# AbeelLab/phasm

Hardware: AMD Instinct MI355X
Metric: overlaps_per_sec (higher is better)
Workload: dtype u64

## Files before the change

phasm_amd/csrc/c_api.hip:

```cpp
#include "../../include/phasm_overlap.h"

#include <hip/hip_runtime.h>

#include <dlfcn.h>
#include <execinfo.h>
#include <fcntl.h>
#include <signal.h>
#include <sys/mman.h>
#include <sys/stat.h>
#include <unistd.h>

#include <algorithm>
#include <array>
#include <atomic>
#include <chrono>
#include <cmath>
#include <condition_variable>
#include <cstdio>
#include <cstdlib>
#include <cstring>
#include <deque>
#include <functional>
#include <memory>
#include <mutex>
// ... 610 lines not shown


unsigned cpu_share() {
    static const unsigned share = [] {
        unsigned n = std::thread::hardware_concurrency();
        n = n ? n : 4u;
        long long q = -1, per = 100000;
        if (FILE* f = std::fopen("/sys/fs/cgroup/cpu.max", "r")) {
            char buf[64] = {0};
            if (std::fscanf(f, "%63s %lld", buf, &per) >= 1 && std::strcmp(buf, "max") != 0) q = atoll(buf);
            std::fclose(f);
        } else if (FILE* g = std::fopen("/sys/fs/cgroup/cpu/cpu.cfs_quota_us", "r")) {
            if (std::fscanf(g, "%lld", &q) != 1) q = -1;
            std::fclose(g);
            if (FILE* g2 = std::fopen("/sys/fs/cgroup/cpu/cpu.cfs_period_us", "r")) {
                if (std::fscanf(g2, "%lld", &per) != 1) per = 100000;
                std::fclose(g2);
            }
        }
        if (q > 0 && per > 0) n = std::min<unsigned>(n, (unsigned)std::max<long long>(1, q / per));
        return n;
    }();
    return share;
}

namespace home {

constexpr uint32_t CHUNK = 4096;

struct Job {
    const void* rec = nullptr;
    uint32_t sh_b = 0, sh_p = 0;
    uint64_t n_rec = 0;
    po_row* out = nullptr;
    uint64_t n_rows = 0;
    const volatile uint32_t* flag = nullptr;
    uint32_t want = 0;
    uint32_t paired = 0, bits = 2;
};

struct Pool {
    std::vector<std::thread> thr;
    std::mutex mu;
    std::condition_variable cv_queue;
    std::condition_variable cv_job;
    std::mutex call_mu;
    std::deque<Job> queue;
    std::atomic<uint64_t> submitted{0}, finished{0};
    std::atomic<int> error{0};
    const uint32_t* len = nullptr;
    uint32_t n_reads = 0;
    std::atomic<uint64_t> sum_l{0}, sum_b{0}, sum_e{0};
    Job cur;
    uint64_t job_seq = 0;
    uint32_t n_chunks = 0;
    std::vector<uint64_t> chunk_off;
    std::atomic<uint32_t> next_count{0}, done_count{0}, next_write{0}, done_write{0};
    std::atomic<int> phase{0};
    std::atomic<int> inside{0};
    std::chrono::steady_clock::time_point t0;
    std::vector<std::array<double, 3>> trace;
    bool tracing = false;
};

Pool* g_pool = nullptr;
std::once_flag g_pool_once;

inline void cpu_pause() {
#if defined(__x86_64__) || defined(__i386__)
    __builtin_ia32_pause();
#endif
}

std::atomic<uint32_t> g_spin_limit{4096};
template <class Pred>
inline void spin_until(Pred pred) {
    const uint32_t limit = g_spin_limit.load(std::memory_order_relaxed);
    for (uint32_t n = 0; !pred(); ++n) {
        if (limit == 0 || n < limit) cpu_pause();
        else std::this_thread::yield();
    }
}

inline po::Cand load_rec(const Job& j, uint64_t i) {
    if (!j.sh_b) return static_cast<const po::Cand*>(j.rec)[i];
    return po::unpack_record(static_cast<const uint64_t*>(j.rec)[i], j.sh_b, j.sh_p);
}

inline uint32_t rows_of_rec(const po::Cand& c, uint32_t paired) {
    if (!paired) return (c.type & 1u) + ((c.type >> 1) & 1u);
    return ((c.type & 1u) ? (c.a == (c.b ^ 1u) ? 1u : 2u) : 0u) + ((c.type & 2u) ? 2u : 0u);
}

inline void put_row(uint64_t*& o, uint32_t a, uint32_t b, uint32_t astart, uint32_t aend, uint32_t bend) {
    __builtin_nontemporal_store((uint64_t)a | ((uint64_t)b << 32), o);
    __builtin_nontemporal_store((uint64_t)astart | ((uint64_t)aend << 32), o + 1);
    __builtin_nontemporal_store((uint64_t)bend << 32, o + 2);
    o += 3;
}

bool expand_records(Pool& P, uint64_t lo, uint64_t hi, po_row* out) {
    uint64_t* o = reinterpret_cast<uint64_t*>(out);
    const Job& job = P.cur;
    const uint32_t* len = P.len;
    const uint32_t paired = job.paired, n_reads = P.n_reads, bits = job.bits;
    auto pb = [bits](uint32_t l) -> uint64_t { return bits == 8u ? l : (l >> 2) + ((l & 3u) != 0u); };
    uint64_t sl = 0, sb = 0, se = 0;
    for (uint64_t i = lo; i < hi; ++i) {
        const po::Cand c = load_rec(job, i);
        if (c.a >= n_reads || c.b >= n_reads) return false;
        const uint32_t la = len[c.a], lb = len[c.b];
        se += 2 * pb((c.type & 1u) ? la - c.p : lb);
        if (c.type & 1u) {
            const uint32_t l = la - c.p;
            const bool twin = paired && c.a != (c.b ^ 1u);
            put_row(o, c.a, c.b, c.p, la, l);
            if (twin) put_row(o, c.b ^ 1u, c.a ^ 1u, lb - l, lb, l);
            const uint64_t k = twin ? 2 : 1;
            sl += k * l;
            sb += k * 2 * pb(l);
        }
        if (c.type & 2u) {
            put_row(o, c.a, c.b, c.p, c.p + lb, lb);
            if (paired) put_row(o, c.a ^ 1u, c.b ^ 1u, la - c.p - lb, la - c.p, lb);
            const uint64_t k = paired ? 2 : 1;
            sl += k * lb;
            sb += k * 2 * pb(lb);
        }
    }
    P.sum_l.fetch_add(sl, std::memory_order_relaxed);
    P.sum_b.fetch_add(sb, std::memory_order_relaxed);
    P.sum_e.fetch_add(se, std::memory_order_relaxed);
    return true;
}

void run_phases(Pool& P, bool lead) {
    const uint32_t nc = P.n_chunks;
    for (;;) {
        const uint32_t c = P.next_count.fetch_add(1, std::memory_order_relaxed);
        if (c >= nc) break;
        const uint64_t lo = (uint64_t)c * CHUNK, hi = std::min<uint64_t>(P.cur.n_rec, lo + CHUNK);
        uint64_t n = 0;
        const uint32_t paired = P.cur.paired;
        for (uint64_t i = lo; i < hi; ++i) n += rows_of_rec(load_rec(P.cur, i), paired);
        P.chunk_off[c + 1] = n;
        P.done_count.fetch_add(1, std::memory_order_release);
    }
    if (lead) {
        spin_until([&] { return P.done_count.load(std::memory_order_acquire) >= nc; });
        P.chunk_off[0] = 0;
        for (uint32_t c = 0; c < nc; ++c) P.chunk_off[c + 1] += P.chunk_off[c];
        if (P.chunk_off[nc] != P.cur.n_rows) P.error.store(1);
        P.phase.store(P.error.load() ? 0 : 2, std::memory_order_release);
    } else {
        spin_until([&] { return P.phase.load(std::memory_order_acquire) != 1; });
    }
    if (P.phase.load(std::memory_order_acquire) != 2) return;
    for (;;) {
        const uint32_t c = P.next_write.fetch_add(1, std::memory_order_relaxed);
        if (c >= nc) break;
        const uint64_t lo = (uint64_t)c * CHUNK, hi = std::min<uint64_t>(P.cur.n_rec, lo + CHUNK);
        if (!expand_records(P, lo, hi, P.cur.out + P.chunk_off[c])) P.error.store(2);
#if defined(__x86_64__)
        __builtin_ia32_sfence();
#endif
        P.done_write.fetch_add(1, std::memory_order_release);
    }
}

void helper(Pool* Pp) {
    Pool& P = *Pp;
    uint64_t seen = 0;
    for (;;) {
        {
            std::unique_lock<std::mutex> lock(P.mu);
            P.cv_job.wait(lock, [&] { return P.job_seq != seen; });
            seen = P.job_seq;
        }
        P.inside.fetch_add(1, std::memory_order_acq_rel);
        if (P.phase.load(std::memory_order_acquire) != 0) run_phases(P, false);
        P.inside.fetch_sub(1, std::memory_order_release);
    }
}

void leader(Pool* Pp) {
    Pool& P = *Pp;
    for (;;) {
        Job j;
        {
            std::unique_lock<std::mutex> lock(P.mu);
            P.cv_queue.wait(lock, [&] { return !P.queue.empty(); });
            j = P.queue.front();
            P.queue.pop_front();
        }
        if (j.flag)
            spin_until([&] { return *j.flag == j.want; });
        std::atomic_thread_fence(std::memory_order_acquire);
        const double t_ready = P.tracing ? std::chrono::duration<double, std::micro>(std::chrono::steady_clock::now() - P.t0).count() : 0.0;
        if (P.error.load() == 0 && j.n_rec) {
            spin_until([&] { return P.inside.load(std::memory_order_acquire) == 0; });
            P.cur = j;
            P.n_chunks = (uint32_t)((j.n_rec + CHUNK - 1) / CHUNK);
            if (P.chunk_off.size() < (size_t)P.n_chunks + 1) P.chunk_off.resize((size_t)P.n_chunks + 1);
            P.next_count.store(0);
            P.done_count.store(0);
            P.next_write.store(0);
            P.done_write.store(0);
            P.phase.store(1, std::memory_order_release);
            {
                std::lock_guard<std::mutex> lock(P.mu);
                ++P.job_seq;
            }
            P.cv_job.notify_all();
            run_phases(P, true);
            if (P.phase.load() == 2)
                spin_until([&] { return P.done_write.load(std::memory_order_acquire) >= P.n_chunks; });
            P.phase.store(0, std::memory_order_release);
            std::atomic_thread_fence(std::memory_order_seq_cst);
        }
        if (P.tracing)
            P.trace.push_back({t_ready, std::chrono::duration<double, std::micro>(std::chrono::steady_clock::now() - P.t0).count(), (double)j.n_rows});
        P.finished.fetch_add(1, std::memory_order_release);
    }
}

Pool* pool() {
    std::call_once(g_pool_once, [] {
        Pool* P = new Pool();
        unsigned n = cpu_share();
        n = std::max(1u, std::min(n * 3 / 4, 12u));
        if (const char* e = getenv("PHASM_HOME_THREADS")) n = (unsigned)std::max(1, std::min(64, atoi(e)));
        try {
            P->thr.emplace_back(leader, P);
            P->thr.back().detach();
            for (unsigned i = 1; i < n; ++i) {
                P->thr.emplace_back(helper, P);
                P->thr.back().detach();
            }
        } catch (const std::system_error&) {
        }
        if (P->thr.empty()) {
            delete P;
            P = nullptr;
        }
        g_pool = P;
    });
    return g_pool;
}

void begin(Pool* P, const uint32_t* len, uint32_t n_reads, bool tracing) {
    if (const char* e = getenv("PHASM_HOME_SPIN")) g_spin_limit.store((uint32_t)std::max(0, atoi(e)));
    else g_spin_limit.store(4096);
    P->len = len;
    P->n_reads = n_reads;
    P->error.store(0);
    P->submitted.store(0);
    P->finished.store(0);
    P->sum_l.store(0);
    P->sum_b.store(0);
    P->sum_e.store(0);
    P->tracing = tracing;
    P->trace.clear();
    P->t0 = std::chrono::steady_clock::now();
}

void submit(Pool* P, const Job& j) {
    {
        std::lock_guard<std::mutex> lock(P->mu);
        P->queue.push_back(j);
    }
    P->submitted.fetch_add(1, std::memory_order_release);
    P->cv_queue.notify_one();
}

void wait_all(Pool* P) {
    spin_until([&] { return P->finished.load(std::memory_order_acquire) >= P->submitted.load(std::memory_order_acquire); });
}

}

po_status init_device(po_handle* h) {
    if (h->dev_ready) {
        HIP_TRY(h, hipSetDevice(h->device));
        return PO_OK;
    }
    AllocTrace tr("init_device", 0);
    const auto ti0 = std::chrono::steady_clock::now();
    auto imark = [&](const char* what) {
        if (tr.on) std::fprintf(stderr, "[init] %s at %.1f ms\n", what, std::chrono::duration<double, std::milli>(std::chrono::steady_clock::now() - ti0).count());
    };
    int n = 0;
    hipError_t e = hipGetDeviceCount(&n);
    imark("runtime up (hipGetDeviceCount)");
    if (e != hipSuccess || n == 0)
        return fail(h, PO_ERR_HIP, "no HIP device available (libphasm_overlap has no CPU fallback)");
    if (h->device < 0 || h->device >= n) return fail(h, PO_ERR_INVALID, "device ordinal out of range");
    HIP_TRY(h, hipSetDevice(h->device));
    hipDeviceProp_t prop;
    HIP_TRY(h, hipGetDeviceProperties(&prop, h->device));
    h->n_cu = prop.multiProcessorCount > 0 ? prop.multiProcessorCount : 256;
// ... 934 lines not shown
            hipLaunchKernelGGL(k_cfill, dim3(cdiv(n_entries, 256)), dim3(256), 0, st, read_slot, entry_off,
                               (uint64_t)n_entries, slot_start, slot_cur, chain64, len);
            sort_chains<uint64_t>();
            hipLaunchKernelGGL(k_fin, dim3(cdiv(nslots, 256)), dim3(256), 0, st, table, nslots, slot_cnt,
                               slot_start, chain64, len);
        }
        HIP_TRY(h, hipGetLastError());
        if (phase_events) HIP_TRY(h, hipEventRecord(h->ev[EV_INDEX], st));
        if (slice_build) {
            HIP_TRY(h, hipStreamSynchronize(st));
            h->sl_tbits = tbits;
            h->sl_entries = h->pinned[0];
            if (phase_events) (void)hipEventElapsedTime(&S.ms_index, h->ev[EV_START], h->ev[EV_INDEX]);
            return PO_OK;
        }
        h->idx_valid = a.idx_only || !ext_idx;
        h->idx_gen = h->upload_gen;
        h->idx_m = m;
        h->idx_wide = wide;
        h->idx_tbits = tbits;
        h->idx_bits = (uint32_t)BITS;
        h->idx_ww = ww;
        *done = a.idx_only;
        return PO_OK;
    }

    po_status scan_count() {
        A.words = words;
        A.tiles = h->d_tiles.as<po::TileRec>();
        A.tile_begin = tile_begin;
        A.tile_end = tile_end;
        A.m = m;
        A.kmask = kmask;
        A.bloom = bloom;
        A.bloom_log2 = bloom_log2;
        A.table = table;
        A.tbits = tbits;
        A.chain = chain;
        A.len = len;
        A.paired = paired;
        A.selfrep = selfrep;
        A.n_selfrep = reinterpret_cast<uint32_t*>(scalars + 2);
        A.tile_count = h->d_tile_count.as<uint32_t>();
        A.tile_off = tile_off_p;
        A.truemask = h->d_truemask.as<uint32_t>();
#ifdef PO_STAMPS
        PO_TRY(ws(h->d_flag, (size_t)4096 * 64));
        HIP_TRY(h, hipMemsetAsync(h->d_flag.p, 0, (size_t)4096 * 64, st));
        A.dbg = h->d_flag.as<unsigned long long>();
#endif
        WA.words = words;
        WA.tiles = A.tiles;
        WA.tile_begin = tile_begin;
        WA.tile_end = tile_end;
        WA.m = m;
        WA.table = table;
        WA.tbits = tbits;
        WA.chain = h->d_chain.as<uint64_t>();
        WA.n_slices = 1;
        if (ext_idx) {
            WA.table = static_cast<const po::Slot*>(a.ext_index);
            WA.chain = nullptr;
            WA.n_slices = a.ext_slices;
            WA.chunk_slots = a.ext_chunk_slots;
            WA.chain_off_slots = a.ext_chain_off;
        }
        WA.len = len;
        WA.paired = paired;
        WA.tile_count = A.tile_count;
        WA.lane_slot = A.truemask;
        WA.tile_off = A.tile_off;
        if (wide) {
            if (pair_events) HIP_TRY(h, hipEventRecord(h->ev[EV_PROBE0], st));
            auto wscan = a.streamed ? (ww == 4 ? po::k_wide_scan<BITS, false, BITS == 2, 4> : po::k_wide_scan<BITS, false, BITS == 2, 1>)
                         : ww == 16 ? po::k_wide_scan<BITS, false, false, 16> : ww == 4 ? po::k_wide_scan<BITS, false, false, 4> : po::k_wide_scan<BITS, false, false, 1>;
            hipLaunchKernelGGL(wscan, dim3(cdiv(ntiles, 4)), dim3(256), 0, st, WA, po::CandGuard{nullptr, 0u});
            if (pair_events) HIP_TRY(h, hipEventRecord(h->ev[EV_PROBE1], st));
        } else {
            const size_t scan_lds = (size_t)scan_waves * po::SCAN_LDS_PER_WAVE + bloom_bytes;
            if (scan_lds > h->lds_max) return fail(h, PO_ERR_HIP, "device LDS too small for the scan kernel");
            constexpr bool CAN_STREAM = BITS == 2;
            auto probe_full = a.streamed ? po::k_scan_probe<BITS, true, CAN_STREAM> : po::k_scan_probe<BITS, true, false>;
            auto probe_part = a.streamed ? po::k_scan_probe<BITS, false, CAN_STREAM> : po::k_scan_probe<BITS, false, false>;
            HIP_TRY(h, hipFuncSetAttribute(reinterpret_cast<const void*>(probe_full), hipFuncAttributeMaxDynamicSharedMemorySize, (int)scan_lds));
            HIP_TRY(h, hipFuncSetAttribute(reinterpret_cast<const void*>(probe_part), hipFuncAttributeMaxDynamicSharedMemorySize, (int)scan_lds));
            const uint32_t n_scan_waves = scan_grid * scan_waves;
            PO_TRY(ws(h->d_left, (size_t)n_scan_waves * po::LEFT_CAP * sizeof(uint2)));
            PO_TRY(ws(h->d_left_cnt, (size_t)n_scan_waves * 4));
            PO_TRY(ws(h->d_tile_extra, ((size_t)h->n_tiles + 1) * 4));
            if (fold_clear && self_clean && h->st_selfclean) {
            } else if (fold_clear) {
                const uint32_t te0 = self_clean ? 0u : tile_begin, ten = self_clean ? h->n_tiles : ntiles;
                hipLaunchKernelGGL(po::k_call_reset, dim3(cdiv(std::max(std::max(n, 16u), std::max(n_scan_waves, ten)), 256)), dim3(256), 0, st,
                                   selfrep, n, self_clean ? h->d_scalars.as<unsigned long long>() : scalars, self_clean ? 16u : 8u,
                                   h->d_left_cnt.as<uint32_t>(), n_scan_waves, h->d_tile_extra.as<uint32_t>() + te0, ten);
            } else {
                HIP_TRY(h, hipMemsetAsync(h->d_left_cnt.p, 0, (size_t)n_scan_waves * 4, st));
                HIP_TRY(h, hipMemsetAsync(h->d_tile_extra.as<uint32_t>() + tile_begin, 0, (size_t)ntiles * 4, st));
            }
            A.left = h->d_left.as<uint2>();
            A.left_cnt = h->d_left_cnt.as<uint32_t>();
            A.tile_extra = h->d_tile_extra.as<uint32_t>();
            if (pair_events) HIP_TRY(h, hipEventRecord(h->ev[EV_PROBE0], st));
            hipLaunchKernelGGL(K == W ? probe_full : probe_part, dim3(scan_grid), dim3(scan_waves * 64), scan_lds, st, A);
            if (pair_events) HIP_TRY(h, hipEventRecord(h->ev[EV_PROBE1], st));
            auto fixup = a.streamed ? po::k_scan_fixup<BITS, CAN_STREAM> : po::k_scan_fixup<BITS, false>;
            hipLaunchKernelGGL(fixup, dim3(n_scan_waves), dim3(256), 0, st, A, n_scan_waves, self_clean ? 1u : 0u);
            if (sw.debug_left) {
                PO_TRY(ensure_host(h, h->scratch_host, (size_t)n_scan_waves * 4));
                HIP_TRY(h, hipMemcpyAsync(h->scratch_host.p, h->d_left_cnt.p, (size_t)n_scan_waves * 4, hipMemcpyDeviceToHost, st));
                HIP_TRY(h, hipStreamSynchronize(st));
                const uint32_t* lc = static_cast<const uint32_t*>(h->scratch_host.p);
                uint64_t sum = 0;
                uint32_t mx = 0;
                for (uint32_t k = 0; k < n_scan_waves; ++k) sum += lc[k], mx = std::max(mx, lc[k]);
                std::fprintf(stderr, "[left] %u scan waves deferred %llu positions (max %u per wave, cap %d)\n", n_scan_waves,
                             (unsigned long long)sum, mx, (int)po::LEFT_CAP);
            }
        }
        HIP_TRY(h, hipGetLastError());
#ifdef PO_STAMPS
        if (!wide) {
            std::vector<unsigned long long> dbg(4096 * 8);
            HIP_TRY(h, hipMemcpyAsync(dbg.data(), h->d_flag.p, dbg.size() * 8, hipMemcpyDeviceToHost, st));
            HIP_TRY(h, hipStreamSynchronize(st));
            double sum[6] = {0, 0, 0, 0, 0, 0};
            for (size_t w = 0; w < 4096; ++w) for (int k = 0; k < 6; ++k) sum[k] += (double)dbg[w * 8 + k];
            if (sum[5] > 0)
                std::fprintf(stderr, "[stamps] per pass (cycles): wait_rw %.0f  filter %.0f  wait_probe %.0f  consume %.0f  issue %.0f  (passes %.0f)\n",
                             sum[0] / sum[5], sum[1] / sum[5], sum[2] / sum[5], sum[3] / sum[5], sum[4] / sum[5], sum[5]);
        }
#endif
        return PO_OK;
    }

    po_status candidate_count() {
        if (a.streamed && h->st_harvest && h->st_pred_valid && !a.dp && !a.want_cands && !sw.sync_count && !sw.tail_classic) {
            uint64_t pred = h->st_pred_cand[a.shard];
            uint64_t cap = pred + pred / 50 + 256;
            if (sw.pred_scale) cap = pred = (uint64_t)((double)pred * atof(sw.pred_scale));
            const uint64_t worst = cap * 4u;
            bool order = pred >= 400000 && (r_end - r_begin) >= 4096;
            if (sw.verify_order) order = atoi(sw.verify_order) != 0;
            pred_order = order;
            auto fits = [](const DevBuf& b, uint64_t bytes) { return b.p && b.cap >= bytes; };
            async_count = pred > 0 && cap < (16u << 20) && cdiv(cap, po::TAIL_TILE) <= po::TAIL_MAX_TILES &&
                          fits(h->d_cand_a, cap * 4) && fits(h->d_cand_p, cap * 4) && fits(h->d_cand_b, cap * 4) && fits(h->d_type, cap) &&
                          fits(h->d_rowcnt, cap) && fits(h->d_row_off, (cap + 1) * 4) &&
                          fits(h->spare_rows, h->home_on ? cap * sizeof(po::Cand) : worst * sizeof(po_row)) &&
                          (!order || (fits(h->d_vlabel, (uint64_t)(r_end - r_begin) * 4) && fits(h->d_vperm, (uint64_t)(r_end - r_begin) * 4) &&
                                      fits(h->d_vrank, (uint64_t)(r_end - r_begin) * 4))) && h->dev_words < 0xFFFFFFF0ull;
            cap_c = (uint32_t)cap;
        }
        volatile uint64_t* count_slot = async_count ? &h->pinned[zone + 8] : &h->pinned[1];
        volatile uint64_t* also_slot = async_count ? &h->pinned[zone + 9] : &h->pinned[8];
        if (ntiles <= po::PS_SMALL_MAX) {
            PO_TRY(prefix_sum_small(h, A.tile_count + tile_begin, wide ? nullptr : A.tile_extra + tile_begin, ntiles,
                                    tile_off_p + tile_begin, count_slot,
                                    reinterpret_cast<const uint64_t*>(scalars + 2), also_slot, st, reinterpret_cast<uint64_t*>(scalars)));
        } else {
            PO_TRY(prefix_sum<uint32_t>(h, A.tile_count + tile_begin, ntiles, tile_off_p + tile_begin, count_slot,
                                        reinterpret_cast<const uint64_t*>(scalars + 2), also_slot,
                                        wide ? nullptr : A.tile_extra + tile_begin, st, reinterpret_cast<uint64_t*>(scalars), a));
        }
        if (phase_events) HIP_TRY(h, hipEventRecord(h->ev[EV_COUNT], st));
        if (async_count) {
            n_cand64 = cap_c;
            n_selfrep_reads = 0;
// ... 5068 lines not shown
```

phasm_amd/csrc/kernels.hip.h:

```cpp
#pragma once
#include <hip/hip_runtime.h>
#include <stdint.h>

namespace po {

using u32x4 = __attribute__((ext_vector_type(4))) uint32_t;

constexpr uint32_t NO_SELFREP = 0xFFFFFFFFu;
constexpr uint64_t KEY_EMPTY = ~0ull;
constexpr int WAVE = 64;

#ifndef PO_VER_PAD
#define PO_VER_PAD 0
#endif
#ifndef PO_SCAN_PAD
#define PO_SCAN_PAD 0
#endif
template <int N>
__device__ __forceinline__ void valu_pad(uint32_t& r, uint32_t c) {
#pragma unroll
    for (int i = 0; i < N; ++i) asm volatile("v_xor_b32 %0, %0, %1" : "+v"(r) : "v"(c));
}

struct CandGuard {
// ... 711 lines not shown
        uint32_t T[48];
        auto make_T = [&](int s) __attribute__((always_inline)) {
            const int j = (2 * s) >> 5, sh = (2 * s) & 31;
            T[s] = sh ? __builtin_amdgcn_alignbit(x[j + 1], x[j], sh) : x[j];
        };
        typedef uint32_t __attribute__((ext_vector_type(2))) u32x2;
        typedef const u32x2 __attribute__((address_space(3))) lds_u32x2;
        auto block_of = [&](int s) __attribute__((always_inline)) -> u32x2 {
            const uint32_t addr = FULLK ? (T[s + 1] & amask) : (((T[s] & klo) >> 2) & amask);
            return *reinterpret_cast<lds_u32x2*>((uintptr_t)addr);
        };
        static_assert(PO_FILTER_DEPTH >= 1 && PO_FILTER_DEPTH <= 16, "the T window below reaches 17 bases ahead");
        u32x2 blk[PO_FILTER_DEPTH];
#pragma unroll
        for (int s = 0; s <= 16; ++s) make_T(s);
#pragma unroll
        for (int s = 0; s < PO_FILTER_DEPTH; ++s) blk[s] = block_of(s);
        __builtin_amdgcn_sched_barrier(0);
#pragma unroll
        for (int s = 0; s < 32; ++s) {
            if (s + 17 < 48) make_T(s + 17);
            const uint32_t t1 = T[s] & klo, t2 = T[s + 16] & khi;
            const uint32_t sel2 = FULLK ? T[s + 10] : (t1 >> 20);
            const u32x2 b = blk[s % PO_FILTER_DEPTH];
            hitmask = __builtin_amdgcn_alignbit((b.x >> (t1 & 31)) & (b.x >> (sel2 & 31)) & (b.y >> (t2 & 31)), hitmask, 1);
            if (s + PO_FILTER_DEPTH < 32) blk[s % PO_FILTER_DEPTH] = block_of(s + PO_FILTER_DEPTH);
            if constexpr (PO_SCAN_PAD > 0) valu_pad<PO_SCAN_PAD>(hitmask, 0u);
            asm volatile("" : "+v"(hitmask));
            __builtin_amdgcn_sched_barrier(0);
        }
    } else {
        const uint32_t wshift = 32 - (bloom_log2 - 5);
#pragma unroll
        for (int s = 0; s < W; ++s) {
            const uint64_t kmer = FULLK ? window<BITS>(w0, w1, s) : (window<BITS>(w0, w1, s) & kmask);
            const uint32_t lo = (uint32_t)kmer, hi = (uint32_t)(kmer >> 32);
            const uint32_t h1 = (lo ^ ((hi << 13) | (hi >> 19))) * 0x9E3779B1u;
            const uint32_t bm = (1u << ((h1 >> 7) & 31)) | (1u << ((h1 >> 12) & 31)) | (1u << ((h1 >> 2) & 31));
            const uint32_t bw = s_bloom[h1 >> wshift];
            hitmask |= ((bw & bm) == bm ? 1u : 0u) << s;
        }
    }
    return hitmask;
}

template <bool STREAM = false, typename F>
__device__ inline void for_each_candidate(const uint32_t* __restrict__ chain, const uint32_t* __restrict__ len,
                                          uint32_t paired, uint32_t z, uint32_t w, uint32_t a, uint32_t rem, F&& f) {
    if (w & SLOT_SINGLE) {
        const uint32_t lb = w & ~SLOT_SINGLE;
        const uint32_t k = keep_bits<STREAM>(a, z, rem, lb, paired);
        if (k) f(z, lb, k);
    } else {
        for (uint32_t j = 0; j < w; ++j) {
            const uint32_t b = chain[z + j];
            const uint32_t lb = len[b];
            const uint32_t k = keep_bits<STREAM>(a, b, rem, lb, paired);
            if (k) f(b, lb, k);
        }
    }
}

#ifndef PO_LEFT_CAP
#define PO_LEFT_CAP 2048
#endif
constexpr uint32_t LEFT_CAP = PO_LEFT_CAP;
constexpr int SCAN_LDS_PER_WAVE = 2 * WAVE * 4 + WAVE * 4;
#ifdef PO_STAMPS
#define PO_STAMP(var) do { __builtin_amdgcn_sched_barrier(0); asm volatile("s_memtime %0\n\ts_waitcnt lgkmcnt(0)" : "=s"(var) :: "memory"); __builtin_amdgcn_sched_barrier(0); } while (0)
#else
#define PO_STAMP(var) do { } while (0)
#endif

template <int BITS, bool FULLK, bool STREAM = false>
__global__ __launch_bounds__(SCAN_BLOCK) void k_scan_probe(const ScanArgs A) {
    constexpr int W = 64 / BITS;
    extern __shared__ uint64_t smem[];
    const uint32_t nwaves = blockDim.x >> 6;
    const uint32_t lane = lane_id(), wave = threadIdx.x >> 6;
    const uint32_t bloom_words = (1u << A.bloom_log2) >> 5;
    uint32_t* s_bloom = reinterpret_cast<uint32_t*>(smem);
    uint32_t* qs = s_bloom + bloom_words + wave * (2 * WAVE);
    uint32_t* tm = s_bloom + bloom_words + (2 * nwaves + wave) * WAVE;
    for (uint32_t i = threadIdx.x; i < bloom_words; i += blockDim.x) s_bloom[i] = A.bloom[i];
    tm[lane] = 0;
    __syncthreads();

    const uint32_t stride = gridDim.x * nwaves;
    const uint32_t tbits = A.tbits, tmask = (1u << A.tbits) - 1u;
    const Slot* __restrict__ table = A.table;
    const uint32_t* __restrict__ chain = A.chain;
    const uint32_t* __restrict__ len = A.len;
    const uint64_t* __restrict__ words = A.words;
    const TileRec* __restrict__ tiles = A.tiles;
    uint32_t* __restrict__ selfrep = A.selfrep;
    uint32_t* __restrict__ n_selfrep = A.n_selfrep;
    uint32_t* __restrict__ truemask = A.truemask;
    uint32_t* __restrict__ tile_count = A.tile_count;
    const uint32_t paired = A.paired, m = A.m, tile_end = A.tile_end;
    const uint64_t kmask = A.kmask;

    uint64_t pk = 0;
    u32x4 ps0 = {0, 0, 0, 0}, ps1 = {0, 0, 0, 0}, ps2 = {0, 0, 0, 0}, ps3 = {0, 0, 0, 0};
    uint32_t pidx = 0, psrc = 0;
    bool pon = false;
    uint64_t pk2 = 0;
    u32x4 pt0 = {0, 0, 0, 0}, pt1 = {0, 0, 0, 0}, pt2 = {0, 0, 0, 0}, pt3 = {0, 0, 0, 0};
    uint32_t pidx2 = 0, psrc2 = 0;
    bool pon2 = false, extra = false;
    uint32_t prev_t = 0xFFFFFFFFu, prev_a = 0, prev_la = 0, prev_word0 = 0;

    auto count_slot = [&](u32x4 s, uint32_t a, uint32_t la, uint32_t p) __attribute__((always_inline)) -> uint32_t {
        uint32_t n = 0;
        if (p > 0) {
            if (s.w & SLOT_SINGLE) {
                if (s.z == a) note_selfrep(selfrep, a, p, n_selfrep);
            } else {
                for (uint32_t j = 0; j < s.w; ++j)
                    if (chain[s.z + j] == a) note_selfrep(selfrep, a, p, n_selfrep);
            }
        }
        for_each_candidate<STREAM>(chain, len, paired, s.z, s.w, a, la - p, [&](uint32_t, uint32_t, uint32_t) { ++n; });
        return n;
    };
    uint2* __restrict__ my_left = A.left + (size_t)(blockIdx.x * nwaves + wave) * LEFT_CAP;
    uint32_t left_n = 0;
    auto defer = [&](bool want, uint32_t tile, uint32_t lane_s) __attribute__((always_inline)) -> bool {
        const uint64_t bal = __ballot(want);
        if (bal == 0) return false;
        const uint32_t cnt = (uint32_t)__popcll(bal);
        if (left_n + cnt > LEFT_CAP) return false;
        if (want) my_left[left_n + (uint32_t)__popcll(bal & ((1ull << lane) - 1ull))] = uint2{tile, lane_s};
        left_n = __builtin_amdgcn_readfirstlane(left_n + cnt);
        return want;
    };

    const uint32_t t_last = tile_end - 1;
    uint32_t t = __builtin_amdgcn_readfirstlane(A.tile_begin + blockIdx.x * nwaves + wave);
    if (t >= tile_end) return;
    auto ld16 = [](const void* ptr) __attribute__((always_inline)) -> u32x4 {
        u32x4 v;
        asm volatile("global_load_dwordx4 %0, %1, off" : "=v"(v) : "v"(ptr) : "memory");
        return v;
    };
    TileRec rec = tiles[t];
    u32x4 r_lo, r_hi, wa, wb = {0, 0, 0, 0};
    {
        const TileRec* rp = &tiles[__builtin_amdgcn_readfirstlane(min(t + stride, t_last))];
        r_lo = ld16(rp);
        r_hi = ld16(reinterpret_cast<const char*>(rp) + 16);
        wa = ld16(&words[rec.wabs + lane]);
        ps0 = ld16(&table[0]);
        ps1 = ld16(&table[1]);
        ps2 = ld16(&table[2]);
        ps3 = ld16(&table[3]);
    }
#ifdef PO_STAMPS
    unsigned long long acc_s[6] = {0, 0, 0, 0, 0, 0};
#endif
    auto pass = [&](u32x4& wcur, u32x4& wnext) __attribute__((always_inline)) -> bool {
        const bool have_tile = t < tile_end;
        const uint32_t tn = t + stride;
        unsigned long long st0 = 0, st1 = 0, st2 = 0, st3 = 0, st4 = 0, st5 = 0;
        (void)st0; (void)st1; (void)st2; (void)st3; (void)st4; (void)st5;
        PO_STAMP(st0);
        asm volatile("s_cmp_eq_u32 %3, 0\n\ts_cbranch_scc1 .Lpo_w4_%=\n\ts_waitcnt vmcnt(8)\n\ts_branch .Lpo_wd_%=\n"
                     ".Lpo_w4_%=:\n\ts_waitcnt vmcnt(4)\n.Lpo_wd_%=:"
// ... 1736 lines not shown
```

Baseline: 1.569 billion.

## Specialize host record expansion, cache LDS attribute, batch bloom filter LDS loads

The host expansion and counting loops are templated on the packed-record flag, and a fast path handles groups of eight plain paired twin records with straight-line stores. This removes per-record branching on the CPU side. The hipFuncSetAttribute call for dynamic LDS size is cached per device and kernel variant, so it is no longer issued on every launch. In the scan probe kernel, the bloom filter copy into LDS uses 128-bit vector loads batched eight deep to get more loads in flight. Some atomics are also tightened to seq_cst, which adds a small synchronization cost.

Result: no change. 1.561 billion (-0.5%).

```diff
diff --git a/phasm_amd/csrc/c_api.hip b/phasm_amd/csrc/c_api.hip
--- a/phasm_amd/csrc/c_api.hip
+++ b/phasm_amd/csrc/c_api.hip
@@ -716,14 +716,28 @@
     }
 }
 
-inline po::Cand load_rec(const Job& j, uint64_t i) {
-    if (!j.sh_b) return static_cast<const po::Cand*>(j.rec)[i];
+template <bool PACKED>
+inline po::Cand load_rec_t(const Job& j, uint64_t i) {
+    if (!PACKED) return static_cast<const po::Cand*>(j.rec)[i];
     return po::unpack_record(static_cast<const uint64_t*>(j.rec)[i], j.sh_b, j.sh_p);
 }
 
 inline uint32_t rows_of_rec(const po::Cand& c, uint32_t paired) {
     if (!paired) return (c.type & 1u) + ((c.type >> 1) & 1u);
     return ((c.type & 1u) ? (c.a == (c.b ^ 1u) ? 1u : 2u) : 0u) + ((c.type & 2u) ? 2u : 0u);
+}
+
+constexpr uint32_t GROUP = 8;
+static_assert(CHUNK % GROUP == 0, "a chunk is a whole number of groups");
+
+inline bool plain_twin(const po::Cand& c) { return (c.type == 1u) & (c.a != (c.b ^ 1u)); }
+
+template <bool PACKED>
+uint64_t count_rows_t(const Job& job, uint64_t lo, uint64_t hi) {
+    const uint32_t paired = job.paired;
+    uint64_t n = 0;
+    for (uint64_t i = lo; i < hi; ++i) n += rows_of_rec(load_rec_t<PACKED>(job, i), paired);
+    return n;
 }
 
 inline void put_row(uint64_t*& o, uint32_t a, uint32_t b, uint32_t astart, uint32_t aend, uint32_t bend) {
@@ -733,39 +747,79 @@
     o += 3;
 }
 
-bool expand_records(Pool& P, uint64_t lo, uint64_t hi, po_row* out) {
+template <bool PACKED>
+bool expand_records_t(Pool& P, uint64_t lo, uint64_t hi, po_row* out) {
     uint64_t* o = reinterpret_cast<uint64_t*>(out);
     const Job& job = P.cur;
     const uint32_t* len = P.len;
     const uint32_t paired = job.paired, n_reads = P.n_reads, bits = job.bits;
     auto pb = [bits](uint32_t l) -> uint64_t { return bits == 8u ? l : (l >> 2) + ((l & 3u) != 0u); };
+    const uint32_t pb_add = bits == 8u ? 0u : 3u, pb_sh = bits == 8u ? 0u : 2u;
     uint64_t sl = 0, sb = 0, se = 0;
-    for (uint64_t i = lo; i < hi; ++i) {
-        const po::Cand c = load_rec(job, i);
-        if (c.a >= n_reads || c.b >= n_reads) return false;
-        const uint32_t la = len[c.a], lb = len[c.b];
-        se += 2 * pb((c.type & 1u) ? la - c.p : lb);
-        if (c.type & 1u) {
-            const uint32_t l = la - c.p;
-            const bool twin = paired && c.a != (c.b ^ 1u);
-            put_row(o, c.a, c.b, c.p, la, l);
-            if (twin) put_row(o, c.b ^ 1u, c.a ^ 1u, lb - l, lb, l);
-            const uint64_t k = twin ? 2 : 1;
-            sl += k * l;
-            sb += k * 2 * pb(l);
-        }
-        if (c.type & 2u) {
-            put_row(o, c.a, c.b, c.p, c.p + lb, lb);
-            if (paired) put_row(o, c.a ^ 1u, c.b ^ 1u, la - c.p - lb, la - c.p, lb);
-            const uint64_t k = paired ? 2 : 1;
-            sl += k * lb;
-            sb += k * 2 * pb(lb);
+    uint64_t i = lo;
+    while (i < hi) {
+        if (paired && i + GROUP <= hi) {
+            uint32_t plain = 1;
+            for (uint32_t k = 0; k < GROUP; ++k) {
+                const po::Cand c = load_rec_t<PACKED>(job, i + k);
+                plain &= (uint32_t)plain_twin(c) & (uint32_t)(c.a < n_reads) & (uint32_t)(c.b < n_reads);
+            }
+            if (plain) {
+                uint64_t gl = 0, gp = 0;
+                for (uint32_t k = 0; k < GROUP; ++k) {
+                    const po::Cand c = load_rec_t<PACKED>(job, i + k);
+                    const uint32_t la = len[c.a], lb = len[c.b], l = la - c.p;
+                    const uint64_t w0 = (uint64_t)c.a | ((uint64_t)c.b << 32), w1 = (uint64_t)c.p | ((uint64_t)la << 32), w2 = (uint64_t)l << 32;
+                    const uint64_t w3 = (uint64_t)(c.b ^ 1u) | ((uint64_t)(c.a ^ 1u) << 32), w4 = (uint64_t)(lb - l) | ((uint64_t)lb << 32);
+                    __builtin_nontemporal_store(w0, o);
+                    __builtin_nontemporal_store(w1, o + 1);
+                    __builtin_nontemporal_store(w2, o + 2);
+                    __builtin_nontemporal_store(w3, o + 3);
+                    __builtin_nontemporal_store(w4, o + 4);
+                    __builtin_nontemporal_store(w2, o + 5);
+                    o += 6;
+                    gl += l;
+                    gp += ((uint64_t)l + pb_add) >> pb_sh;
+                }
+                sl += 2 * gl;
+                sb += 4 * gp;
+                se += 2 * gp;
+                i += GROUP;
+                continue;
+            }
+        }
+        const uint64_t stop = std::min<uint64_t>(hi, i + GROUP);
+        for (; i < stop; ++i) {
+            const po::Cand c = load_rec_t<PACKED>(job, i);
+            if (c.a >= n_reads || c.b >= n_reads) return false;
+            const uint32_t la = len[c.a], lb = len[c.b];
+            se += 2 * pb((c.type & 1u) ? la - c.p : lb);
+            if (c.type & 1u) {
+                const uint32_t l = la - c.p;
+                const bool twin = paired && c.a != (c.b ^ 1u);
+                put_row(o, c.a, c.b, c.p, la, l);
+                if (twin) put_row(o, c.b ^ 1u, c.a ^ 1u, lb - l, lb, l);
+                const uint64_t k = twin ? 2 : 1;
+                sl += k * l;
+                sb += k * 2 * pb(l);
+            }
+            if (c.type & 2u) {
+                put_row(o, c.a, c.b, c.p, c.p + lb, lb);
+                if (paired) put_row(o, c.a ^ 1u, c.b ^ 1u, la - c.p - lb, la - c.p, lb);
+                const uint64_t k = paired ? 2 : 1;
+                sl += k * lb;
+                sb += k * 2 * pb(lb);
+            }
         }
     }
     P.sum_l.fetch_add(sl, std::memory_order_relaxed);
     P.sum_b.fetch_add(sb, std::memory_order_relaxed);
     P.sum_e.fetch_add(se, std::memory_order_relaxed);
     return true;
+}
+
+bool expand_records(Pool& P, uint64_t lo, uint64_t hi, po_row* out) {
+    return P.cur.sh_b ? expand_records_t<true>(P, lo, hi, out) : expand_records_t<false>(P, lo, hi, out);
 }
 
 void run_phases(Pool& P, bool lead) {
@@ -774,10 +828,7 @@
         const uint32_t c = P.next_count.fetch_add(1, std::memory_order_relaxed);
         if (c >= nc) break;
         const uint64_t lo = (uint64_t)c * CHUNK, hi = std::min<uint64_t>(P.cur.n_rec, lo + CHUNK);
-        uint64_t n = 0;
-        const uint32_t paired = P.cur.paired;
-        for (uint64_t i = lo; i < hi; ++i) n += rows_of_rec(load_rec(P.cur, i), paired);
-        P.chunk_off[c + 1] = n;
+        P.chunk_off[c + 1] = P.cur.sh_b ? count_rows_t<true>(P.cur, lo, hi) : count_rows_t<false>(P.cur, lo, hi);
         P.done_count.fetch_add(1, std::memory_order_release);
     }
     if (lead) {
@@ -811,8 +862,9 @@
             P.cv_job.wait(lock, [&] { return P.job_seq != seen; });
             seen = P.job_seq;
         }
-        P.inside.fetch_add(1, std::memory_order_acq_rel);
-        if (P.phase.load(std::memory_order_acquire) != 0) run_phases(P, false);
+        P.inside.fetch_add(1, std::memory_order_seq_cst);
+        std::atomic_thread_fence(std::memory_order_seq_cst);
+        if (P.phase.load(std::memory_order_seq_cst) != 0) run_phases(P, false);
         P.inside.fetch_sub(1, std::memory_order_release);
     }
 }
@@ -832,7 +884,7 @@
         std::atomic_thread_fence(std::memory_order_acquire);
         const double t_ready = P.tracing ? std::chrono::duration<double, std::micro>(std::chrono::steady_clock::now() - P.t0).count() : 0.0;
         if (P.error.load() == 0 && j.n_rec) {
-            spin_until([&] { return P.inside.load(std::memory_order_acquire) == 0; });
+            spin_until([&] { return P.inside.load(std::memory_order_seq_cst) == 0; });
             P.cur = j;
             P.n_chunks = (uint32_t)((j.n_rec + CHUNK - 1) / CHUNK);
             if (P.chunk_off.size() < (size_t)P.n_chunks + 1) P.chunk_off.resize((size_t)P.n_chunks + 1);
@@ -849,7 +901,7 @@
             run_phases(P, true);
             if (P.phase.load() == 2)
                 spin_until([&] { return P.done_write.load(std::memory_order_acquire) >= P.n_chunks; });
-            P.phase.store(0, std::memory_order_release);
+            P.phase.store(0, std::memory_order_seq_cst);
             std::atomic_thread_fence(std::memory_order_seq_cst);
         }
         if (P.tracing)
@@ -1950,8 +2002,18 @@
             constexpr bool CAN_STREAM = BITS == 2;
             auto probe_full = a.streamed ? po::k_scan_probe<BITS, true, CAN_STREAM> : po::k_scan_probe<BITS, true, false>;
             auto probe_part = a.streamed ? po::k_scan_probe<BITS, false, CAN_STREAM> : po::k_scan_probe<BITS, false, false>;
-            HIP_TRY(h, hipFuncSetAttribute(reinterpret_cast<const void*>(probe_full), hipFuncAttributeMaxDynamicSharedMemorySize, (int)scan_lds));
-            HIP_TRY(h, hipFuncSetAttribute(reinterpret_cast<const void*>(probe_part), hipFuncAttributeMaxDynamicSharedMemorySize, (int)scan_lds));
+            {
+                constexpr int MAX_DEV = 64;
+                static std::atomic<uint32_t> lds_set[MAX_DEV][2][2] = {};
+                std::atomic<uint32_t>* have = h->device >= 0 && h->device < MAX_DEV ? &lds_set[h->device][K == W ? 1 : 0][a.streamed && CAN_STREAM ? 1 : 0] : nullptr;
+                if (!have || have->load(std::memory_order_acquire) < (uint32_t)scan_lds) {
+                    HIP_TRY(h, hipFuncSetAttribute(reinterpret_cast<const void*>(K == W ? probe_full : probe_part),
+                                                   hipFuncAttributeMaxDynamicSharedMemorySize, (int)scan_lds));
+                    uint32_t seen = have ? have->load(std::memory_order_relaxed) : 0u;
+                    while (have && seen < (uint32_t)scan_lds && !have->compare_exchange_weak(seen, (uint32_t)scan_lds, std::memory_order_release)) {
+                    }
+                }
+            }
             const uint32_t n_scan_waves = scan_grid * scan_waves;
             PO_TRY(ws(h->d_left, (size_t)n_scan_waves * po::LEFT_CAP * sizeof(uint2)));
             PO_TRY(ws(h->d_left_cnt, (size_t)n_scan_waves * 4));
diff --git a/phasm_amd/csrc/kernels.hip.h b/phasm_amd/csrc/kernels.hip.h
--- a/phasm_amd/csrc/kernels.hip.h
+++ b/phasm_amd/csrc/kernels.hip.h
@@ -817,7 +817,22 @@
     uint32_t* s_bloom = reinterpret_cast<uint32_t*>(smem);
     uint32_t* qs = s_bloom + bloom_words + wave * (2 * WAVE);
     uint32_t* tm = s_bloom + bloom_words + (2 * nwaves + wave) * WAVE;
-    for (uint32_t i = threadIdx.x; i < bloom_words; i += blockDim.x) s_bloom[i] = A.bloom[i];
+    {
+        constexpr uint32_t FILTER_BATCH = 8;
+        const uint32_t bloom_vecs = bloom_words >> 2;
+        const u32x4* __restrict__ gsrc = reinterpret_cast<const u32x4*>(A.bloom);
+        u32x4* sdst = reinterpret_cast<u32x4*>(smem);
+        for (uint32_t base = threadIdx.x; base < bloom_vecs; base += FILTER_BATCH * blockDim.x) {
+            u32x4 v[FILTER_BATCH];
+#pragma unroll
+            for (uint32_t k = 0; k < FILTER_BATCH; ++k) v[k] = gsrc[min(base + k * blockDim.x, bloom_vecs - 1u)];
+#pragma unroll
+            for (uint32_t k = 0; k < FILTER_BATCH; ++k) asm volatile("" : "+v"(v[k]));
+#pragma unroll
+            for (uint32_t k = 0; k < FILTER_BATCH; ++k)
+                if (base + k * blockDim.x < bloom_vecs) sdst[base + k * blockDim.x] = v[k];
+        }
+    }
     tm[lane] = 0;
     __syncthreads();
 
```
